# krisher/PathTracer.cl

Measured on AMD Instinct MI355X. Metric: Mrays/sec + frames/sec at 1920×1080, 871k-tri PLY, 1/2/4/8 MI355X, higher is better.
Workload: dtype f32

## Files before the change

__graft_entry__.py:

```python
from __future__ import annotations

import os
import subprocess
import sys
from pathlib import Path

ROOT = Path(__file__).resolve().parent


def _make(path: Path, *targets: str) -> None:
    jobs = str(min(16, os.cpu_count() or 1))
    subprocess.run(["make", "-s", "-j", jobs, "-C", str(path), *targets], check=True)


def build() -> None:
    _make(ROOT / "pathtracer.cl_amd" / "csrc")
    _make(ROOT / "oracle")
    sys.path.insert(0, str(ROOT / "oracle"))
    from oracle import REFERENCE_ROOT

    if os.access(REFERENCE_ROOT / "clrt" / "ocl" / "raytracer.cl", os.R_OK):
        _make(ROOT / "oracle", "ref")
        _make(ROOT / "tests" / "cpp", "all", "libdevkat.so")
    else:
        _make(ROOT / "tests" / "cpp", "ref_main_replay", "host_tree_dump", "libdevkat.so")
    sys.path.insert(0, str(ROOT))
    import ptload

    pt = ptload.load()
    pt.load_library()


def smoke() -> None:
    import numpy as np

    sys.path.insert(0, str(ROOT))
    sys.path.insert(0, str(ROOT / "oracle"))
    import ptload
    from oracle import Oracle

    pt = ptload.load()
    sc = pt.scenes
    orc = Oracle()
    W, H, sr = 64, 48, 2
    Wp, Hp = sc.padded_dims(W, H)
    verts, idx = sc.make_mesh(4000)
    seeds = sc.default_seeds(Wp, Hp)

# ... 43 lines not shown
```

include/pathtracer_rt.h:

```cpp
#ifndef PATHTRACER_RT_H
#define PATHTRACER_RT_H

#include <stddef.h>
#include <stdint.h>

#include "rt_types.h"

#ifdef __cplusplus
extern "C" {
#endif

typedef struct rt_ctx rt_ctx;

enum {
    RT_OK = 0,
    RT_ERR_ARG = -1,
    RT_ERR_HIP = -2,
    RT_ERR_NO_SCENE = -3,
    RT_ERR_NO_MESH = -4,
    RT_ERR_ALLOC = -5,
    RT_ERR_STATE = -6,
    RT_ERR_LIMIT = -7
};

// ... 35 lines not shown
    uint64_t pixel_steps_max;
    uint64_t rays_skipped;
    uint64_t clocks_shade;
    uint64_t pixels_long;
} rt_counters;

int rt_create(int device, rt_ctx **out);
int rt_destroy(rt_ctx *ctx);
const char *rt_last_error(const rt_ctx *ctx);
const char *rt_status_string(int status);

int rt_set_spheres(rt_ctx *ctx, const rt_sphere *spheres, uint32_t n);

int rt_set_mesh(rt_ctx *ctx, const float *verts_xyz, uint32_t n_verts, const int32_t *idx, uint32_t n_tris);
typedef struct rt_mesh_stats {
    uint32_t n_tris;
    uint32_t n_nodes2, depth2;
    uint32_t n_nodes4, depth4;
    uint32_t stack4;
    double build_seconds;
    uint32_t builder;
    uint32_t n_tris_tree;
    uint32_t n_nodes4_shadow;
} rt_mesh_stats;
enum { RT_BUILD_HOST = 0, RT_BUILD_GPU = 1 };
int rt_set_builder(rt_ctx *ctx, int builder);
int rt_mesh_info(const rt_ctx *ctx, rt_mesh_stats *out);

enum { RT_MESH_VERTS_DEVICE = 1 };
enum { RT_MESH_UPDATE_REFIT = 1, RT_MESH_UPDATE_REBUILT = 2 };
enum { RT_REFIT_OK = 0, RT_REFIT_NEWLY_HITTABLE = 1, RT_REFIT_ENCODING = 2 };
typedef struct rt_mesh_update_info {
    uint32_t action;
    uint32_t reason;
    uint32_t newly_hittable;
    uint32_t now_unhittable;
    float area_ratio;
    float ms;
} rt_mesh_update_info;
int rt_update_mesh(rt_ctx *ctx, const float *verts_xyz, uint32_t n_verts, int flags);
int rt_last_mesh_update(const rt_ctx *ctx, rt_mesh_update_info *out);
int rt_set_mesh_dynamic(rt_ctx *ctx, int on);
int rt_mesh_pose(rt_ctx *ctx, float *out_verts_xyz, uint32_t n_verts, int flags);

int rt_set_view_matrix(rt_ctx *ctx, const float m_colmajor[16]);
int rt_set_camera_spherical(rt_ctx *ctx, float tx, float ty, float tz, float elevation_deg, float azimuth_deg,
// ... 31 lines not shown
int rt_last_kernel_ms(const rt_ctx *ctx, float *ms);
int rt_last_kernel_split_ms(const rt_ctx *ctx, float *prepass_ms, float *main_ms);

typedef struct rt_render_info {
    uint32_t kernel;
    uint32_t traversal;
    uint32_t grid_blocks;
    uint32_t lists;
    uint64_t list_capacity;
    uint64_t list_records;
    uint32_t list_pixels_tree;
    uint32_t pixels_long;
    uint32_t schedule_rebuilt;
    uint32_t lists_rebuilt;
    double schedule_host_ms;
    uint32_t split_chunks;
    uint32_t split_coop;
    uint32_t split_guard;
    uint32_t split_spec;
    uint32_t split_repaired;
    uint32_t split_hit_depth;
    uint32_t schedule_measured;
    uint32_t schedule_pilot;
} rt_render_info;
int rt_last_render_info(rt_ctx *ctx, rt_render_info *out);
int rt_last_long_chains(rt_ctx *ctx, uint32_t *out, uint32_t cap, uint32_t *n);
int rt_last_list_counts(rt_ctx *ctx, uint16_t *out, uint32_t cap, uint32_t *n);
typedef struct rt_tree_layout {
    uint32_t n_nodes4;
    uint32_t n_nodes4_shadow;
    uint32_t shadow_root;
    uint32_t n_records;
    uint32_t compressed;
} rt_tree_layout;
int rt_mesh_tree(rt_ctx *ctx, rt_tree_layout *layout, float *nodes4, uint32_t *nodes4q, float *tris);

int rt_trace_rays(rt_ctx *ctx, const rt_ray *rays, uint32_t n, int any_hit, int32_t *out_idx, float *out_t);

enum { RT_FEAT_BOX = -1, RT_FEAT_NONE = -2, RT_FEAT_SPHERE0 = -16  };
int rt_get_camera(const rt_ctx *ctx, uint32_t width, rt_camera *out);
int rt_primary_rays(const rt_camera *cam, uint32_t width, uint32_t height, rt_ray *out);
int rt_render_features(rt_ctx *ctx, float *feat, uint32_t width, uint32_t height, int kernel, int flags);
int rt_render_features_async(rt_ctx *ctx, float *feat, uint32_t width, uint32_t height, int kernel, int flags,
                             void *hip_stream);
typedef struct rt_denoise_params {
    uint32_t iterations;
// ... 113 lines not shown
```

pathtracer.cl_amd/_abi.py:

```python
from __future__ import annotations

import ctypes
import os
from pathlib import Path

import numpy as np

PKG_DIR = Path(__file__).resolve().parent
LIB_PATH = PKG_DIR / "librtmi.so"

RT_OK = 0
RT_ERR_ARG = -1
RT_ERR_HIP = -2
RT_ERR_NO_SCENE = -3
RT_ERR_NO_MESH = -4
RT_ERR_ALLOC = -5
RT_ERR_STATE = -6
RT_ERR_LIMIT = -7

RT_KERNEL_SPHERES = 0
RT_KERNEL_SPHERES_SS = 1
RT_KERNEL_TRIS = 2

RT_TRAVERSAL_BVH = 0
# ... 52 lines not shown
CAMERA_FLOATS = 16


class RtTile(ctypes.Structure):
    _fields_ = [("stripe_rows", ctypes.c_uint32), ("n_ranks", ctypes.c_uint32), ("rank", ctypes.c_uint32),
                ("stripe_owner", ctypes.c_void_p)]


def tile_struct(tile):
    if tile is None:
        return None, None
    stripe, n, r = (int(v) for v in tile[:3])
    owner = tile[3] if len(tile) > 3 else None
    if owner is None:
        return RtTile(stripe, n, r, None), None
    o = np.ascontiguousarray(owner, np.uint32)
    return RtTile(stripe, n, r, o.ctypes.data), o


class RtMeshStats(ctypes.Structure):
    _fields_ = [("n_tris", ctypes.c_uint32), ("n_nodes2", ctypes.c_uint32), ("depth2", ctypes.c_uint32),
                ("n_nodes4", ctypes.c_uint32), ("depth4", ctypes.c_uint32), ("stack4", ctypes.c_uint32),
                ("build_seconds", ctypes.c_double), ("builder", ctypes.c_uint32), ("n_tris_tree", ctypes.c_uint32),
                ("n_nodes4_shadow", ctypes.c_uint32)]


class RtMeshUpdateInfo(ctypes.Structure):
    _fields_ = [("action", ctypes.c_uint32), ("reason", ctypes.c_uint32), ("newly_hittable", ctypes.c_uint32),
                ("now_unhittable", ctypes.c_uint32), ("area_ratio", ctypes.c_float), ("ms", ctypes.c_float)]


class RtTreeLayout(ctypes.Structure):
    _fields_ = [("n_nodes4", ctypes.c_uint32), ("n_nodes4_shadow", ctypes.c_uint32), ("shadow_root", ctypes.c_uint32),
                ("n_records", ctypes.c_uint32), ("compressed", ctypes.c_uint32)]


class RtCounters(ctypes.Structure):
    _fields_ = [
        ("rays_closest", ctypes.c_uint64),
        ("rays_shadow", ctypes.c_uint64),
        ("nodes_visited", ctypes.c_uint64),
        ("tris_tested", ctypes.c_uint64),
        ("leaves_visited", ctypes.c_uint64),
        ("lane_slots", ctypes.c_uint64),
        ("clocks_traversal", ctypes.c_uint64),
        ("clocks_total", ctypes.c_uint64),
        ("pixel_clocks_max", ctypes.c_uint64),
# ... 6 lines not shown


class RtRenderInfo(ctypes.Structure):
    _fields_ = [
        ("kernel", ctypes.c_uint32),
        ("traversal", ctypes.c_uint32),
        ("grid_blocks", ctypes.c_uint32),
        ("lists", ctypes.c_uint32),
        ("list_capacity", ctypes.c_uint64),
        ("list_records", ctypes.c_uint64),
        ("list_pixels_tree", ctypes.c_uint32),
        ("pixels_long", ctypes.c_uint32),
        ("schedule_rebuilt", ctypes.c_uint32),
        ("lists_rebuilt", ctypes.c_uint32),
        ("schedule_host_ms", ctypes.c_double),
        ("split_chunks", ctypes.c_uint32),
        ("split_coop", ctypes.c_uint32),
        ("split_guard", ctypes.c_uint32),
        ("split_spec", ctypes.c_uint32),
        ("split_repaired", ctypes.c_uint32),
        ("split_hit_depth", ctypes.c_uint32),
        ("schedule_measured", ctypes.c_uint32),
        ("schedule_pilot", ctypes.c_uint32),
    ]


class RtDenoiseParams(ctypes.Structure):
    _fields_ = [("iterations", ctypes.c_uint32), ("sigma_color", ctypes.c_float), ("sigma_normal", ctypes.c_float),
                ("sigma_plane", ctypes.c_float)]


class RtReprojectParams(ctypes.Structure):
    _fields_ = [("plane_tol", ctypes.c_float), ("normal_min", ctypes.c_float), ("max_history", ctypes.c_float)]


class RtTrustParams(ctypes.Structure):
    _fields_ = [("tolerance", ctypes.c_float), ("sigma_normal", ctypes.c_float), ("sigma_plane", ctypes.c_float)]


class RtDenoiseVarParams(ctypes.Structure):
    _fields_ = [("iterations", ctypes.c_uint32), ("sigma_lum", ctypes.c_float), ("sigma_normal", ctypes.c_float),
                ("sigma_plane", ctypes.c_float), ("min_len", ctypes.c_float)]


_vp, _u32, _i32, _f32, _sz = ctypes.c_void_p, ctypes.c_uint32, ctypes.c_int, ctypes.c_float, ctypes.c_size_t
SIGNATURES = {
# ... 146 lines not shown
```

pathtracer.cl_amd/csrc/rt_bvh.cpp:

```cpp
#include <algorithm>
#include <array>
#include <functional>
#include <chrono>
#include <cmath>
#include <cstdlib>
#include <cstring>
#include <string>
#include <vector>

#include "rt_internal.h"
#include "rt_quant.h"

namespace {

struct Box {
    float lo[3], hi[3];
    void reset()
    {
        for (int k = 0; k < 3; ++k) {
            lo[k] = INFINITY;
            hi[k] = -INFINITY;
        }
    }
    void grow(const Box &b)
// ... 209 lines not shown
    }
    for (uint64_t i = 0; i < 3ull * n_tris; ++i) {
        if (idx[i] < 0 || (uint32_t)idx[i] >= n_verts) {
            err = "vertex index out of range";
            return false;
        }
    }
    return true;
}

static bool never_hit(const float *a, const float *p1, const float *p2)
{
    const float e1[3] = {p1[0] - a[0], p1[1] - a[1], p1[2] - a[2]};
    const float e2[3] = {p2[0] - a[0], p2[1] - a[1], p2[2] - a[2]};
    const double cx = (double)e2[1] * e1[2] - (double)e2[2] * e1[1];
    const double cy = (double)e2[2] * e1[0] - (double)e2[0] * e1[2];
    const double cz = (double)e2[0] * e1[1] - (double)e2[1] * e1[0];
    const double cr = std::sqrt(cx * cx + cy * cy + cz * cz);
    const double n1 = std::fabs((double)e1[0]) + std::fabs((double)e1[1]) + std::fabs((double)e1[2]);
    const double n2 = std::fabs((double)e2[0]) + std::fabs((double)e2[1]) + std::fabs((double)e2[2]);
    const double u = 1.0 / 16777216.0;
    const double bound = 1.001 * (cr + 16.0 * u * n1 * n2);
    return bound < 0.999 * (double)1e-4f;
}

bool rt_build_bvh(const float *verts, uint32_t n_verts, const int32_t *idx, uint32_t n_tris, RtBvh &out,
                  std::string &err)
{
    const auto t0 = std::chrono::steady_clock::now();
    if (!rt_validate_mesh(verts, n_verts, idx, n_tris, err)) return false;

    Builder b;
    b.lights = out.light_centres;
    b.light_w = out.light_cost_weight;
    b.verts = verts;
    b.idx = idx;
    b.tbox.resize(n_tris);
    b.cent.resize(3ull * n_tris);
    b.perm.resize(n_tris);
    for (uint32_t t = 0; t < n_tris; ++t) {
        Box bx;
        bx.reset();
        float maxabs = 0.0f;
        for (int k = 0; k < 3; ++k) {
            const float *p = verts + 3ull * (uint32_t)idx[3ull * t + k];
            bx.grow(p);
            for (int c = 0; c < 3; ++c) maxabs = std::max(maxabs, std::fabs(p[c]));
        }
        float ext = 0.0f;
        for (int c = 0; c < 3; ++c) ext = std::max(ext, bx.hi[c] - bx.lo[c]);
        const float pad = ext * (1.0f / 512.0f) + 1e-6f * (1.0f + maxabs);
        for (int c = 0; c < 3; ++c) {
            b.cent[3ull * t + c] = 0.5f * (bx.lo[c] + bx.hi[c]);
            bx.lo[c] -= pad;
            bx.hi[c] += pad;
        }
        b.tbox[t] = bx;
    }
    uint32_t n_hit = 0;
    if (out.cull_unhittable) {
        std::vector<uint8_t> hit(n_tris);
        for (uint32_t t = 0; t < n_tris; ++t) {
            const float *a = verts + 3ull * (uint32_t)idx[3ull * t];
            const float *p1 = verts + 3ull * (uint32_t)idx[3ull * t + 1];
            const float *p2 = verts + 3ull * (uint32_t)idx[3ull * t + 2];
            hit[t] = !never_hit(a, p1, p2);
            n_hit += hit[t];
        }
        if (n_hit == 0) hit[0] = 1, n_hit = 1;
        for (uint32_t t = 0, k = 0, r = n_hit; t < n_tris; ++t) b.perm[hit[t] ? k++ : r++] = t;
    } else {
        n_hit = n_tris;
        for (uint32_t t = 0; t < n_tris; ++t) b.perm[t] = t;
    }
    out.n_hit = n_hit;
    b.nodes.reserve(2ull * n_hit / RT_LEAF_MAX + 16);
    const int root = b.build(0, n_hit, 1);

    std::vector<int> order;
    std::vector<int> out_index(b.nodes.size(), -1);
    uint32_t n_leaves = 0;
    if (b.nodes[root].left < 0) {
        out.n_nodes = 1;
        out.nodes.assign(16, 0.0f);
        const Box &bx = b.nodes[root].box;
        float *n = out.nodes.data();
        n[0] = bx.lo[0]; n[1] = bx.hi[0]; n[2] = bx.lo[1]; n[3] = bx.hi[1];
        n[4] = bx.lo[0]; n[5] = bx.hi[0]; n[6] = bx.lo[1]; n[7] = bx.hi[1];
        n[8] = bx.lo[2]; n[9] = bx.hi[2]; n[10] = bx.lo[2]; n[11] = bx.hi[2];
        const int32_t code = leaf_code(0, n_hit);
        std::memcpy(&n[12], &code, 4);
        std::memcpy(&n[13], &code, 4);
        n_leaves = 1;
        out.depth = 1;
    } else {
        std::vector<int> stack;
        stack.push_back(root);
        while (!stack.empty()) {
            const int id = stack.back();
            stack.pop_back();
// ... 61 lines not shown
            const int l = nd.left, r = nd.right;
            float best_int = INFINITY;
            for (int a = 1; a <= 3; ++a) best_int = std::min(best_int, dcost[l][a] + dcost[r][4 - a]);
            const float inner_c = area * 1.0f + best_int;
            const float self_c = std::min(leaf_c, inner_c);
            as_leaf[i] = leaf_c <= inner_c;
            dcost[i][1] = self_c;
            dsplit[i][1] = 0;
            for (int j = 2; j <= 4; ++j) {
                float best = self_c;
                int8_t arg = 0;
                for (int a = 1; a < j; ++a) {
                    const float c = dcost[l][a] + dcost[r][j - a];
                    if (c < best) {
                        best = c;
                        arg = (int8_t)a;
                    }
                }
                dcost[i][j] = best;
                dsplit[i][j] = arg;
            }
        }
    }
    {
        std::vector<int> n4_src;
        std::vector<int> kids_of;
        std::function<void(int, int, int *, int &)> expand = [&](int id, int j, int *k, int &n) {
            const int a = dsplit[id][j];
            if (a == 0) {
                k[n++] = id;
                return;
            }
            expand(b.nodes[id].left, a, k, n);
            expand(b.nodes[id].right, j - a, k, n);
        };
        auto gather = [&](int id, int *kids) {
            int k[4] = {-1, -1, -1, -1};
            int n = 0;
            if (b.nodes[id].left < 0) {
                k[n++] = id;
            } else {
                const int l = b.nodes[id].left, r = b.nodes[id].right;
                int best_a = 1;
                float best = INFINITY;
                for (int a = 1; a <= 3; ++a) {
                    const float c = dcost[l][a] + dcost[r][4 - a];
                    if (c < best) {
                        best = c;
                        best_a = a;
                    }
                }
                expand(l, best_a, k, n);
                expand(r, 4 - best_a, k, n);
            }
            for (int i = 0; i < 4; ++i) {
                kids[i] = k[i];
                if (k[i] >= 0) inner4[k[i]] = !as_leaf[k[i]];
            }
        };
        std::vector<int> st{root};
        inner4[root] = b.nodes[root].left >= 0;
        while (!st.empty()) {
            const int id = st.back();
// ... 104 lines not shown
                    c = new_id[c];
                    std::memcpy(&dst[24 + k], &c, 4);
                } else {
                    remap(&dst[24 + k]);
                }
            }
        }
        out.nodes4.swap(nodes4);
        for (uint32_t i = 0; i < out.n_nodes; ++i) {
            remap(&out.nodes[16ull * i + 12]);
            remap(&out.nodes[16ull * i + 13]);
        }
        for (uint32_t q = cursor; q < n_tris; ++q) new_perm[q] = b.perm[q];
        b.perm.swap(new_perm);
    }

    out.nodes4q.assign((uint64_t)RT_QNODE_DWORDS * out.n_nodes4, 0u);
    for (uint32_t i = 0; i < out.n_nodes4; ++i)
        if (!rt_quantize_node4(out.nodes4.data() + 32ull * i, out.nodes4q.data() + (uint64_t)RT_QNODE_DWORDS * i)) {
            out.nodes4q.clear();
            break;
        }

    out.tris.assign(12ull * n_tris, 0.0f);
    for (uint32_t s = 0; s < n_tris; ++s) {
        const uint32_t t = b.perm[s];
        const float *a = verts + 3ull * (uint32_t)idx[3ull * t];
        const float *p1 = verts + 3ull * (uint32_t)idx[3ull * t + 1];
        const float *p2 = verts + 3ull * (uint32_t)idx[3ull * t + 2];
        float *o = out.tris.data() + 12ull * s;
        o[0] = a[0];
        o[1] = a[1];
        o[2] = a[2];
        const int32_t orig = (int32_t)t;
        std::memcpy(&o[3], &orig, 4);
        o[4] = p1[0] - a[0];
        o[5] = p1[1] - a[1];
        o[6] = p1[2] - a[2];
        o[8] = p2[0] - a[0];
        o[9] = p2[1] - a[1];
        o[10] = p2[2] - a[2];
    }
    if (!out.nodes4q.empty() && out.det_cull) {
        struct NB {
            double lo[3], hi[3], err;
        };
// ... 44 lines not shown
```

pathtracer.cl_amd/csrc/rt_ctx.h:

```cpp
#ifndef RT_CTX_H
#define RT_CTX_H

#include <hip/hip_runtime.h>

#include <algorithm>
#include <cstdint>
#include <cstdlib>
#include <string>
#include <utility>
#include <vector>

#include "pathtracer_rt.h"
#include "rt_internal.h"

template <class T> struct DevBuf {
    T *p = nullptr;
    size_t cap = 0;
    DevBuf() = default;
    DevBuf(const DevBuf &) = delete;
    DevBuf &operator=(DevBuf &&o) noexcept
    {
        std::swap(p, o.p);
        std::swap(cap, o.cap);
        return *this;
// ... 37 lines not shown
    }
    operator H() const { return h; }
};
struct Event : Owned<hipEvent_t, hipEventDestroy> {
    hipError_t create(unsigned flags = hipEventDefault) { return h ? hipSuccess : hipEventCreateWithFlags(&h, flags); }
};
struct Stream : Owned<hipStream_t, hipStreamDestroy> {
    hipError_t create() { return h ? hipSuccess : hipStreamCreateWithFlags(&h, hipStreamNonBlocking); }
};

struct GlibcRand {
    uint32_t r[34];
    int k = 0;
    void seed(uint32_t s);
    uint32_t next();
};

constexpr size_t kCounterBytes = RT_COUNTER_WORDS * sizeof(unsigned long long);
constexpr size_t kWorkWords = (size_t)RT_QSTRIDE * RT_QHEADS + 64;
static_assert((kCounterBytes + kWorkWords * sizeof(uint32_t)) % sizeof(unsigned long long) == 0, "d_counters is an array of 64-bit words");
#ifndef RT_REPAIR_SLOTS
#define RT_REPAIR_SLOTS 4096u
#endif

enum RtStage { RT_ST_FEATURES, RT_ST_DENOISE, RT_ST_REPROJECT, RT_ST_MERGE, RT_ST_MOMENTS, RT_ST_VARIANCE, RT_ST_DENOISE_VAR, RT_ST_WARP, RT_ST_TRUST, RT_ST_COUNT };

struct rt_ctx {
    int device = 0;
    hipStream_t stream = nullptr;
    Event ev0, ev1, evm;
    std::string err;

    std::vector<rt_sphere> spheres;
    std::vector<rt_sphere> lights;
    DevBuf<rt_sphere> d_spheres, d_lights;

    RtBvh bvh;
    DevBuf<float> d_nodes4;
    DevBuf<uint32_t> d_nodes4q;
    DevBuf<float> d_tris;
    size_t tris_cap() const { return d_tris.cap / 12; }
    size_t tree_recs = 0;
    uint32_t shadow_root = 0;
    uint32_t n_nodes4_shadow = 0, stack4_all = 0;
    std::vector<std::pair<uint32_t, uint32_t>> shadow_levels;
    bool shadow_cache = true;
    int shadow_cache_depth = -1;
    DevBuf<uint16_t> d_list_code;
    DevBuf<uint32_t> d_list_tile;
    DevBuf<uint32_t> d_list_alloc;
    int pixel_lists = -1;
    size_t list_mb = 4096;
    std::vector<uint32_t> list_key;
    uint64_t list_used_last = 0, list_cap_last = 0, list_npx_last = 0;
    std::vector<uint32_t> last_view;
    uint32_t n_tris = 0;
    DevBuf<int32_t> d_spill;
    DevBuf<uint32_t> d_order;
    DevBuf<uint32_t> d_flags;
    RtSchedScratch sched;
    DevBuf<int32_t> d_class;
    size_t split_mb = 16384;
    int split = -1;
    uint32_t seed_width = 0;
    uint32_t split_probe = 4;
    uint32_t split_nch = 16;
    DevBuf<uint32_t> d_split_seed;
    DevBuf<float> d_split_col;
    DevBuf<uint32_t> d_split_counter;
    DevBuf<uint32_t> d_split_box;
// ... 194 lines not shown
```

pathtracer.cl_amd/csrc/rt_internal.h:

```cpp
#ifndef RT_INTERNAL_H
#define RT_INTERNAL_H

#include <stdint.h>

#include <string>
#include <vector>

#include "rt_types.h"

int rt_exception_status(std::string *err) noexcept;
#define RT_CATCH(err_ptr)                                                                                              \
    catch (...) { return rt_exception_status(err_ptr); }

#ifndef RT_STACK_DEPTH
#define RT_STACK_DEPTH 20
#endif
#define RT_BVH_MAX_DEPTH 33
#define RT_BLOCK 256
#define RT_PROBE_HIT_SHIFT 27
#define RT_PROBE_STEP_MASK ((1u << RT_PROBE_HIT_SHIFT) - 1u)
#ifndef RT_STEP_UNROLL
#define RT_STEP_UNROLL 4
#endif
#ifndef RT_DIAG_ONE_PIXEL
// ... 13 lines not shown
#define RT_CNT_GUARD RT_N_COUNTERS
#define RT_CNT_REPAIR (RT_N_COUNTERS + 1)
#define RT_COUNTER_WORDS (RT_N_COUNTERS + 2)
enum { RT_GUARD_INDEX = 1, RT_GUARD_STACK = 2, RT_GUARD_ROUNDS = 4 };

#define RT_EMPTY_CHILD 0x7fffffff

struct RtBvh {
    std::vector<float> nodes;
    std::vector<float> tris;
    uint32_t n_nodes = 0;
    uint32_t n_leaves = 0;
    uint32_t depth = 0;
    std::vector<float> nodes4;
    std::vector<uint32_t> nodes4q;
    uint32_t n_nodes4 = 0;
    uint32_t depth4 = 0;
    uint32_t stack4 = 0;
    double build_seconds = 0.0;
    bool cull_unhittable = true;
    bool det_cull = true;
    std::vector<float> light_centres;
    float light_cost_weight = 0.6f;
    uint32_t n_hit = 0;
};

bool rt_build_bvh(const float *verts, uint32_t n_verts, const int32_t *idx, uint32_t n_tris, RtBvh &out,
                  std::string &err);

struct RtGpuBvh {
    float *nodes4 = nullptr;
    uint32_t *nodes4q = nullptr;
    float *tris = nullptr;
    uint32_t n_nodes4 = 0, depth4 = 0, stack4 = 0;
    double build_seconds = 0.0;
};
int rt_build_bvh_gpu(const float *verts, uint32_t n_verts, const int32_t *idx, uint32_t n_tris, RtGpuBvh &out,
                     std::string &err, void *stream, bool det_cull = true);
bool rt_validate_mesh(const float *verts, uint32_t n_verts, const int32_t *idx, uint32_t n_tris, std::string &err);

enum {
    RT_REFIT_RES_BAD = 0,
    RT_REFIT_RES_NEWLY = 1,
    RT_REFIT_RES_UNHIT = 2,
    RT_REFIT_RES_QFAIL = 3,
    RT_REFIT_RES_LO = 4,
    RT_REFIT_RES_HI = 7,
// ... 213 lines not shown
```

pathtracer.cl_amd/csrc/rt_mesh.cpp:

```cpp
#include <cmath>
#include <cstring>
#include <thread>

#include "rt_ctx.h"
#include "rt_math.h"
#include "rt_quant.h"

namespace {

std::vector<std::pair<uint32_t, uint32_t>> tree_levels(const uint32_t *q4, uint32_t n, uint32_t root)
{
    std::vector<std::pair<uint32_t, uint32_t>> lv;
    if (!q4 || root >= n) return lv;
    uint32_t lo = root, hi = root + 1u;
    for (;;) {
        lv.emplace_back(lo, hi);
        uint32_t cmin = ~0u, cmax = 0u, cnt = 0u;
        for (uint32_t i = lo; i < hi; ++i)
            for (int k = 0; k < 4; ++k) {
                const int32_t code = (int32_t)q4[(size_t)i * RT_QNODE_DWORDS + 12 + k];
                if (code < 0 || code == RT_EMPTY_CHILD) continue;
                cmin = std::min(cmin, (uint32_t)code);
                cmax = std::max(cmax, (uint32_t)code);
                ++cnt;
            }
        if (!cnt) break;
        if (cmin != hi || cmax - cmin + 1u != cnt || cmax >= n) break;
        lo = cmin;
        hi = cmax + 1u;
    }
    return lv;
}

}

extern "C" {

static bool mesh_bounds(const float *verts, const int32_t *idx, uint32_t n_tris, float lo[3], float hi[3])
{
    for (int k = 0; k < 3; ++k) {
        lo[k] = INFINITY;
        hi[k] = -INFINITY;
    }
    for (uint64_t i = 0; i < 3ull * n_tris; ++i) {
        const float *v = verts + 3ull * (uint32_t)idx[i];
        for (int k = 0; k < 3; ++k) {
            lo[k] = std::min(lo[k], v[k]);
            hi[k] = std::max(hi[k], v[k]);
        }
    }
// ... 26 lines not shown
    drop_mesh(c);
    RtGpuBvh g;
    bool det_cull = true;
    if (const char *v = getenv("RT_DET_CULL")) det_cull = atoi(v) != 0;
    const int e = rt_build_bvh_gpu(verts, n_verts, idx, n_tris, g, err, c->stream, det_cull);
    c->d_nodes4.adopt(g.nodes4, 32ull * g.n_nodes4);
    c->d_nodes4q.adopt(g.nodes4q, (size_t)RT_QNODE_DWORDS * g.n_nodes4);
    c->d_tris.adopt(g.tris, 12ull * n_tris);
    if (e) return fail(c, RT_ERR_HIP, "GPU BVH build: " + err);
    c->n_tris = n_tris;
    c->mesh_serial++;
    c->bvh.n_nodes = 0;
    c->bvh.n_leaves = 0;
    c->bvh.depth = 0;
    c->bvh.n_nodes4 = g.n_nodes4;
    c->bvh.depth4 = g.depth4;
    c->bvh.stack4 = g.stack4;
    c->bvh.build_seconds = g.build_seconds;
    c->bvh.n_hit = n_tris;
    c->tree_recs = n_tris;
    c->shadow_root = 0;
    c->n_nodes4_shadow = 0;
    c->stack4_all = g.stack4;
    c->shadow_levels.clear();
    if (c->shadow_cache && g.nodes4q) {
        std::vector<uint32_t> hq((size_t)RT_QNODE_DWORDS * g.n_nodes4);
        HIPCHK(c, hipMemcpy(hq.data(), g.nodes4q, hq.size() * sizeof(uint32_t), hipMemcpyDeviceToHost));
        c->shadow_levels = tree_levels(hq.data(), g.n_nodes4, 0u);
    }
    c->mesh_builder = RT_BUILD_GPU;
    c->mesh_bounds_ok = mesh_bounds(verts, idx, n_tris, c->mesh_lo, c->mesh_hi);
    c->mesh_det_cull = det_cull;
    c->mesh_dynamic = dynamic;
    return RT_OK;
}

static int set_mesh_build(rt_ctx *c, const float *verts, uint32_t n_verts, const int32_t *idx, uint32_t n_tris,
                          int builder, bool dynamic)
{
    std::string err;
    c->mesh_bounds_ok = false;
    if (builder == RT_BUILD_GPU) return set_mesh_build_gpu(c, verts, n_verts, idx, n_tris, dynamic);
    RtBvh b;
    if (const char *v = getenv("RT_CULL_UNHITTABLE")) b.cull_unhittable = atoi(v) != 0;
    if (dynamic) b.cull_unhittable = false;
    if (const char *v = getenv("RT_DET_CULL")) b.det_cull = atoi(v) != 0;
    RtBvh sb;
    sb.cull_unhittable = b.cull_unhittable;
    sb.det_cull = b.det_cull;
    for (const rt_sphere &L : c->lights) {
        sb.light_centres.push_back(L.center.x);
        sb.light_centres.push_back(L.center.y);
        sb.light_centres.push_back(L.center.z);
    }
    if (const char *v = getenv("RT_BVH_LIGHT_W")) sb.light_cost_weight = (float)atof(v);
    b.light_cost_weight = 0.0f;
    bool two = !sb.light_centres.empty() && sb.light_cost_weight > 0.0f && 2ull * n_tris < (1ull << 28);
    bool ok2 = false;
    std::string err2;
    std::thread th;
    if (two)
        th = std::thread([&]() {
            try {
                ok2 = rt_build_bvh(verts, n_verts, idx, n_tris, sb, err2);
            } catch (...) {
                ok2 = false;
            }
        });
    bool ok = false;
    try {
        ok = rt_build_bvh(verts, n_verts, idx, n_tris, b, err);
    } catch (...) {
        if (th.joinable()) th.join();
        throw;
    }
    if (th.joinable()) th.join();
    if (!ok)
        return fail(c, err.find("deeper") != std::string::npos ? RT_ERR_LIMIT : RT_ERR_ARG, err);
// ... 11 lines not shown
                if (code >= 0) {
                    code += (int32_t)n_a;
                } else {
                    const uint32_t enc = (uint32_t)(~code);
                    code = ~(int32_t)((((enc >> 3) + n_tris) << 3) | (enc & 7u));
                }
                w = (uint32_t)code;
            }
        tr.insert(tr.end(), sb.tris.begin(), sb.tris.end());
    }
    c->mesh_builder = RT_BUILD_HOST;
    drop_mesh(c);
    HIPCHK(c, c->d_nodes4.reserve(b.nodes4.size()));
    if (!q4.empty()) HIPCHK(c, c->d_nodes4q.reserve(q4.size()));
    HIPCHK(c, c->d_tris.reserve(tr.size()));
    HIPCHK(c, hipMemcpy(c->d_nodes4, b.nodes4.data(), b.nodes4.size() * sizeof(float), hipMemcpyHostToDevice));
    if (!q4.empty())
        HIPCHK(c, hipMemcpy(c->d_nodes4q, q4.data(), q4.size() * sizeof(uint32_t), hipMemcpyHostToDevice));
    HIPCHK(c, hipMemcpy(c->d_tris, tr.data(), tr.size() * sizeof(float), hipMemcpyHostToDevice));
    c->tree_recs = tr.size() / 12;
    c->shadow_root = two ? n_a : 0u;
    c->n_nodes4_shadow = two ? sb.n_nodes4 : 0u;
    c->shadow_levels = tree_levels(q4.data(), (uint32_t)(q4.size() / RT_QNODE_DWORDS), c->shadow_root);
    c->stack4_all = two ? std::max(b.stack4, sb.stack4) : b.stack4;
    c->n_tris = n_tris;
    c->mesh_serial++;
    c->bvh.n_nodes = b.n_nodes;
    c->bvh.n_leaves = b.n_leaves;
    c->bvh.depth = b.depth;
    c->bvh.n_nodes4 = b.n_nodes4;
    c->bvh.depth4 = b.depth4;
    c->bvh.stack4 = b.stack4;
    c->bvh.build_seconds = b.build_seconds;
    c->bvh.n_hit = b.n_hit;
    c->mesh_bounds_ok = mesh_bounds(verts, idx, n_tris, c->mesh_lo, c->mesh_hi);
    c->mesh_det_cull = b.det_cull;
    c->mesh_dynamic = dynamic;
    return RT_OK;
}

static int refit_prepare(rt_ctx *c)
{
    rt_ctx::Refit &r = c->refit;
    const uint32_t n_a = c->bvh.n_nodes4, n_s = c->n_nodes4_shadow, n_all = n_a + n_s;
    std::vector<uint32_t> q((size_t)RT_QNODE_DWORDS * n_all, 0u);
    if (c->d_nodes4q) {
// ... 137 lines not shown
    a.nbox = r.d_nbox;
    a.tris = c->d_tris;
    a.tbox = r.d_tbox;
    a.n_nodes4 = n_a;
    a.n_nodes4_shadow = c->n_nodes4_shadow;
    a.n_recs = (uint32_t)c->tree_recs;
    a.det_cull = c->mesh_det_cull;
    a.res = r.d_res;
    HIPCHK(c, hipEventRecord(r.ev0, st));
    if (int e = rt_launch_refit_records(r.d_verts, c->d_idx, n_tris, n_hit, a.n_recs, c->d_tris, r.d_tbox, r.d_hit0,
                                        !r.have_hit0, r.d_res, st))
        return hip_fail(c, (hipError_t)e, "k_refit_records");
    r.have_hit0 = true;
    if (int e = rt_launch_refit_levels(a, r.d_steps, r.steps.data(), (uint32_t)r.steps.size(), st))
        return hip_fail(c, (hipError_t)e, "k_refit_levels");
    double now = 0.0;
    if (int e = rt_launch_refit_area(c->d_nodes4, n_a, r.d_part, st))
        return hip_fail(c, (hipError_t)e, "k_refit_area");
    HIPCHK(c, hipEventRecord(r.ev1, st));
    HIPCHK(c, hipMemcpyAsync(res, r.d_res, sizeof(res), hipMemcpyDeviceToHost, st));
    HIPCHK(c, hipMemcpyAsync(part, r.d_part, sizeof(part), hipMemcpyDeviceToHost, st));
    HIPCHK(c, hipStreamSynchronize(st));
    c->mesh_serial++;
    if (res[RT_REFIT_RES_BAD]) return fail(c, RT_ERR_STATE, "rt_update_mesh: a link of the tree is out of range");
    const bool had_q = c->d_nodes4q != nullptr;
    if (had_q ? res[RT_REFIT_RES_QFAIL] != 0u : res[RT_REFIT_RES_QFAIL] == 0u)
        return update_rebuild(c, verts, flags, RT_REFIT_ENCODING, 0u);
    for (double p : part) now += p;
    float ext = 0.0f;
    for (int k = 0; k < 3; ++k) {
        auto unkey = [](uint32_t key) { return (key & 0x80000000u) ? (key & 0x7FFFFFFFu) : ~key; };
        const uint32_t ul = unkey(res[RT_REFIT_RES_LO + k]), uh = unkey(res[RT_REFIT_RES_HI + k]);
        memcpy(&c->mesh_lo[k], &ul, 4);
        memcpy(&c->mesh_hi[k], &uh, 4);
        ext = std::max(ext, c->mesh_hi[k] - c->mesh_lo[k]);
    }
    const float pad = 1e-3f * ext + 1e-4f;
    for (int k = 0; k < 3; ++k) {
        c->mesh_lo[k] -= pad;
        c->mesh_hi[k] += pad;
    }
    c->mesh_bounds_ok = true;
    if (const int w = wait_aux(c, st)) return w;
    HIPCHK(c, hipMemcpyAsync(c->d_pose, r.d_verts, 12ull * n_verts, hipMemcpyDeviceToDevice, st));
    HIPCHK(c, hipStreamSynchronize(st));
    float ms = 0.0f;
// ... 12 lines not shown
    if (n_verts != c->n_verts) return fail(c, RT_ERR_ARG, "rt_mesh_pose: the vertex count differs from the mesh's");
    if (flags & ~RT_OUT_DEVICE) return fail(c, RT_ERR_ARG, "rt_mesh_pose: flags other than RT_OUT_DEVICE");
    HIPCHK(c, hipSetDevice(c->device));
    HIPCHK(c, hipMemcpy(out, c->d_pose, 12ull * n_verts,
                        (flags & RT_OUT_DEVICE) ? hipMemcpyDeviceToDevice : hipMemcpyDeviceToHost));
    HIPCHK(c, hipStreamSynchronize(nullptr));
    return RT_OK;
} RT_CATCH(err_of(c))

int rt_mesh_info(const rt_ctx *c, rt_mesh_stats *out)
try {
    if (!c || !out) return RT_ERR_ARG;
    if (!c->n_tris) return RT_ERR_NO_MESH;
    out->n_tris = c->n_tris;
    out->n_nodes2 = c->bvh.n_nodes;
    out->depth2 = c->bvh.depth;
    out->n_nodes4_shadow = c->n_nodes4_shadow;
    out->n_nodes4 = c->bvh.n_nodes4;
    out->depth4 = c->bvh.depth4;
    out->stack4 = c->bvh.stack4;
    out->builder = (uint32_t)c->mesh_builder;
    out->build_seconds = c->bvh.build_seconds;
    out->n_tris_tree = c->bvh.n_hit;
    return RT_OK;
} RT_CATCH(err_of(c))

int rt_mesh_tree(rt_ctx *c, rt_tree_layout *layout, float *nodes4, uint32_t *nodes4q, float *tris)
try {
    if (!c || !layout) return RT_ERR_ARG;
    if (!c->n_tris || !c->d_nodes4 || !c->d_tris) return RT_ERR_NO_MESH;
    layout->n_nodes4 = c->bvh.n_nodes4;
    layout->n_nodes4_shadow = c->n_nodes4_shadow;
    layout->shadow_root = c->shadow_root;
    layout->n_records = (uint32_t)c->tree_recs;
    layout->compressed = c->d_nodes4q ? 1u : 0u;
    if (nodes4q && !c->d_nodes4q) return fail(c, RT_ERR_STATE, "the mesh has no compressed nodes");
    if (!nodes4 && !nodes4q && !tris) return RT_OK;
    HIPCHK(c, hipSetDevice(c->device));
    HIPCHK(c, hipStreamSynchronize(c->stream));
    if (nodes4)
        HIPCHK(c, hipMemcpy(nodes4, c->d_nodes4, (size_t)c->bvh.n_nodes4 * 32 * sizeof(float), hipMemcpyDeviceToHost));
    if (nodes4q)
        HIPCHK(c, hipMemcpy(nodes4q, c->d_nodes4q,
                            ((size_t)c->bvh.n_nodes4 + c->n_nodes4_shadow) * RT_QNODE_DWORDS * sizeof(uint32_t),
                            hipMemcpyDeviceToHost));
    if (tris) HIPCHK(c, hipMemcpy(tris, c->d_tris, c->tree_recs * 12 * sizeof(float), hipMemcpyDeviceToHost));
// ... 62 lines not shown
```

pathtracer.cl_amd/csrc/rt_render.cpp:

```cpp
#include <chrono>
#include <cmath>
#include <cstdio>
#include <cstring>

#include "rt_ctx.h"

namespace {

constexpr uint32_t kProbeN = 2;
uint32_t probe_n(uint32_t sample_rate) { return sample_rate >= 2 ? kProbeN : 1u; }
#ifndef RT_FETCH_K
#define RT_FETCH_K 24
#endif
constexpr uint32_t kWorkBox = RT_QSTRIDE * RT_QHEADS, kWorkRepair = RT_QSTRIDE * RT_QHEADS + 32;
#ifndef RT_LONG_FINE
#define RT_LONG_FINE 1
#endif
#ifndef RT_REPAIR_WIDTH
#define RT_REPAIR_WIDTH 64u
#endif
#ifndef RT_QUEUE_BATCH
#define RT_QUEUE_BATCH 64
#endif
#ifndef RT_BOX_GRID_DIV
// ... 461 lines not shown
{
    a.out = f.dout;
    a.seeds = c->d_seeds;
    a.cam = c->cam;
    a.W = f.W;
    a.H = f.H;
    a.Wpad = c->wpad;
    a.Hpad = c->hpad;
    a.Hl = f.hl;
    a.sample_rate = c->sample_rate;
    a.max_depth = c->max_depth;
    a.progressive = f.prog;
    a.stripe = f.stripe;
    a.n_ranks = f.nr;
    a.rank = f.rk;
    a.stripe_map = f.smap;
    a.counters = c->d_counters;
}

int tri_scene(rt_ctx *c, RtTriLaunch &a)
{
    a.nodes = trav_nodes(c);
    a.shadow_root = trav_kind(c) == RT_TRAV_BVH4Q ? c->shadow_root : 0u;
    if (trav_kind(c) == RT_TRAV_BVH4Q && c->shadow_cache) {
        const size_t nl = c->shadow_levels.size();
        const size_t d = c->shadow_cache_depth >= 0 ? (size_t)c->shadow_cache_depth
                                                    : std::min<size_t>(kShadowCutDepth, (nl - (nl > 0)) / 2);
        if (d >= 1 && d < nl && c->shadow_levels[d].second - c->shadow_levels[d].first <= 0xffffu) {
            a.shadow_cut_lo = c->shadow_levels[d].first;
            a.shadow_cut_hi = c->shadow_levels[d].second;
        }
    }
    a.tris = c->d_tris;
    a.n_tris = c->n_tris;
    a.lights = c->d_lights;
    a.n_lights = (uint32_t)c->lights.size();
    if (a.n_lights > 16) return fail(c, RT_ERR_LIMIT, "more than 16 emissive spheres");
    return RT_OK;
}

int plan_grid(rt_ctx *c, const Frame &f, RtTriLaunch &a, TriPlan &p)
{
    const uint64_t items = (uint64_t)((f.W + 7) / 8) * ((f.hl + 7) / 8) * 64;
    p.item_blocks = (items + RT_BLOCK - 1) / RT_BLOCK;
    int r = grid_blocks(c, p.trav, c->counting, RT_FORM_PLAIN, &p.blocks);
    if (r != RT_OK) return r;
    p.blocks = std::max(1, (int)std::min<uint64_t>((uint64_t)p.blocks, p.item_blocks));
    p.short_frame = (uint64_t)f.W * f.hl * c->sample_rate * c->sample_rate <
                    kShortFrameSamplesPerLane * (uint64_t)p.blocks * RT_BLOCK;
    if (p.short_frame) p.blocks = std::max(1, p.blocks * (int)kShortFrameBlocksPerCU / RT_TRIS_WAVES);
    if (const uint32_t gb = env_u32("RTMI_GRID_BLOCKS", 0)) p.blocks = std::min(p.blocks, (int)gb);
    if (p.trav == RT_TRAV_BVH4Q) {
        r = grid_blocks(c, p.trav, c->counting, RT_FORM_SPLIT, &p.blocks_split);
// ... 249 lines not shown
    *e_out = e;
    return RT_OK;
}

void tris_info(rt_ctx *c, const RtTriLaunch &a, const TriPlan &p)
{
    c->info = rt_render_info{};
    c->info.kernel = RT_KERNEL_TRIS;
    c->info.traversal = (uint32_t)p.trav;
    c->info.grid_blocks = (uint32_t)p.blocks;
    c->info.lists = p.lists ? 1u : 0u;
    c->info.lists_rebuilt = p.build_lists ? 1u : 0u;
    c->info.list_capacity = p.lists ? p.list_cap : 0;
    c->info_list_px = p.lists ? (size_t)p.npx : 0u;
    c->info.pixels_long = c->last_long;
    c->info.split_chunks = a.split_chunks;
    c->info.split_coop = a.split_chunks && a.split_n_box ? a.split_coop : 0u;
    c->info.split_spec = a.split_chunks ? a.split_spec : 0u;
    c->info.split_hit_depth = a.split_chunks && c->last_hit_depth ? 1u : 0u;
    c->info.schedule_measured = a.tile_order && c->order_measured ? 1u : 0u;
    c->info.schedule_rebuilt = c->schedule_rebuilt ? 1u : 0u;
    c->info.schedule_host_ms = p.sched_ms;
    c->info.schedule_pilot = p.pilot ? 1u : 0u;
    c->info_list_pending = p.lists;
}

int render_tris(rt_ctx *c, const Frame &f, int *e_out)
{
    RtTriLaunch a{};
    TriPlan p;
    common_fields(a, c, f);
    a.map_key = f.map_key;
    a.work_counter = c->d_work;
    if (const int r = tri_scene(c, a)) return r;
    p.trav = trav_kind(c);
    if (const int r = plan_grid(c, f, a, p)) return r;
    stepping_fields(f, a, p);
    a.tile_order = nullptr;
    a.pixel_flags = nullptr;
    a.pixel_class = nullptr;
    const auto h0 = std::chrono::steady_clock::now();
    c->schedule_rebuilt = false;
    if (c->schedule) {
        const int ro = tile_order(c, a, p.blocks, f.st);
        if (ro != RT_OK) return ro;
        a.tile_order = c->d_order;
// ... 447 lines not shown
```

Measured before the change: 17710.

## Split shadow BVH into a light-cone subtree of potentially occluding triangles

At build time each hittable triangle is tested against every emissive sphere with a conservative cone bound. Triangles whose projected area toward all lights falls below the existing degenerate threshold are flagged as never occluding. The shadow BVH is rebuilt with a root whose left child holds only the occluding triangles, and shadow rays start traversal at that subtree. The aim is to cut shadow-ray node and triangle tests, at the cost of extra host build work, staleness tracking after refits, and a risk of precision mismatch against the oracle.

```diff
diff --git a/__graft_entry__.py b/__graft_entry__.py
--- a/__graft_entry__.py
+++ b/__graft_entry__.py
@@ -24,6 +24,7 @@
         _make(ROOT / "tests" / "cpp", "all", "libdevkat.so")
     else:
         _make(ROOT / "tests" / "cpp", "ref_main_replay", "host_tree_dump", "libdevkat.so")
+    _make(ROOT / "tests" / "cpp", "-f", "light_cone.mk")
     sys.path.insert(0, str(ROOT))
     import ptload
 
diff --git a/include/pathtracer_rt.h b/include/pathtracer_rt.h
--- a/include/pathtracer_rt.h
+++ b/include/pathtracer_rt.h
@@ -81,6 +81,8 @@
     uint32_t builder;
     uint32_t n_tris_tree;
     uint32_t n_nodes4_shadow;
+    uint32_t cone_root;
+    uint32_t n_tris_cone;
 } rt_mesh_stats;
 enum { RT_BUILD_HOST = 0, RT_BUILD_GPU = 1 };
 int rt_set_builder(rt_ctx *ctx, int builder);
@@ -158,6 +160,7 @@
     uint32_t split_hit_depth;
     uint32_t schedule_measured;
     uint32_t schedule_pilot;
+    uint32_t shadow_start;
 } rt_render_info;
 int rt_last_render_info(rt_ctx *ctx, rt_render_info *out);
 int rt_last_long_chains(rt_ctx *ctx, uint32_t *out, uint32_t cap, uint32_t *n);
diff --git a/pathtracer.cl_amd/_abi.py b/pathtracer.cl_amd/_abi.py
--- a/pathtracer.cl_amd/_abi.py
+++ b/pathtracer.cl_amd/_abi.py
@@ -98,7 +98,7 @@
     _fields_ = [("n_tris", ctypes.c_uint32), ("n_nodes2", ctypes.c_uint32), ("depth2", ctypes.c_uint32),
                 ("n_nodes4", ctypes.c_uint32), ("depth4", ctypes.c_uint32), ("stack4", ctypes.c_uint32),
                 ("build_seconds", ctypes.c_double), ("builder", ctypes.c_uint32), ("n_tris_tree", ctypes.c_uint32),
-                ("n_nodes4_shadow", ctypes.c_uint32)]
+                ("n_nodes4_shadow", ctypes.c_uint32), ("cone_root", ctypes.c_uint32), ("n_tris_cone", ctypes.c_uint32)]
 
 
 class RtMeshUpdateInfo(ctypes.Structure):
@@ -151,6 +151,7 @@
         ("split_hit_depth", ctypes.c_uint32),
         ("schedule_measured", ctypes.c_uint32),
         ("schedule_pilot", ctypes.c_uint32),
+        ("shadow_start", ctypes.c_uint32),
     ]
 
 
diff --git a/pathtracer.cl_amd/csrc/rt_bvh.cpp b/pathtracer.cl_amd/csrc/rt_bvh.cpp
--- a/pathtracer.cl_amd/csrc/rt_bvh.cpp
+++ b/pathtracer.cl_amd/csrc/rt_bvh.cpp
@@ -255,6 +255,49 @@
     const double u = 1.0 / 16777216.0;
     const double bound = 1.001 * (cr + 16.0 * u * n1 * n2);
     return bound < 0.999 * (double)1e-4f;
+}
+
+static bool never_occludes(const float *a, const float *p1, const float *p2, const std::vector<float> &centres,
+                           const std::vector<float> &radii)
+{
+    const float e1[3] = {p1[0] - a[0], p1[1] - a[1], p1[2] - a[2]};
+    const float e2[3] = {p2[0] - a[0], p2[1] - a[1], p2[2] - a[2]};
+    const double n[3] = {(double)e2[1] * e1[2] - (double)e2[2] * e1[1], (double)e2[2] * e1[0] - (double)e2[0] * e1[2],
+                         (double)e2[0] * e1[1] - (double)e2[1] * e1[0]};
+    const double cr = std::sqrt(n[0] * n[0] + n[1] * n[1] + n[2] * n[2]);
+    const double n1 = std::fabs((double)e1[0]) + std::fabs((double)e1[1]) + std::fabs((double)e1[2]);
+    const double n2 = std::fabs((double)e2[0]) + std::fabs((double)e2[1]) + std::fabs((double)e2[2]);
+    const double u = 1.0 / 16777216.0;
+    double cen[3], rt2 = 0.0;
+    for (int k = 0; k < 3; ++k) cen[k] = (double)a[k] + ((double)e1[k] + (double)e2[k]) / 3.0;
+    for (int v = 0; v < 3; ++v) {
+        double d2 = 0.0;
+        for (int k = 0; k < 3; ++k) {
+            const double p = (double)a[k] + (v == 1 ? (double)e1[k] : v == 2 ? (double)e2[k] : 0.0);
+            d2 += (p - cen[k]) * (p - cen[k]);
+        }
+        rt2 = std::max(rt2, d2);
+    }
+    const double rt = std::sqrt(rt2);
+    for (size_t l = 0; l < radii.size(); ++l) {
+        double L[3], dist2 = 0.0, ln = 0.0;
+        for (int k = 0; k < 3; ++k) {
+            L[k] = (double)centres[3 * l + k] - cen[k];
+            dist2 += L[k] * L[k];
+            ln += L[k] * n[k];
+        }
+        const double dist = std::sqrt(dist2);
+        const double reach = 1.001 * std::fabs((double)radii[l]) + rt;
+        double maxcos = 1.0;
+        if (reach < dist && cr > 0.0) {
+            const double st = reach / dist, ct = std::sqrt(1.0 - st * st);
+            const double cp = std::min(1.0, std::fabs(ln) / (dist * cr)), sp = std::sqrt(1.0 - cp * cp);
+            if (cp < ct) maxcos = std::min(1.0, (cp * ct + sp * st) * (1.0 + 1e-9) + 1e-12);
+        }
+        const double bound = 1.001 * (cr * maxcos + 16.0 * u * n1 * n2);
+        if (!(bound < 0.999 * (double)1e-4f)) return false;
+    }
+    return true;
 }
 
 bool rt_build_bvh(const float *verts, uint32_t n_verts, const int32_t *idx, uint32_t n_tris, RtBvh &out,
@@ -290,7 +333,9 @@
         }
         b.tbox[t] = bx;
     }
-    uint32_t n_hit = 0;
+    uint32_t n_hit = 0, n_cone = 0;
+    out.cone_root4 = 0;
+    out.n_cone = 0;
     if (out.cull_unhittable) {
         std::vector<uint8_t> hit(n_tris);
         for (uint32_t t = 0; t < n_tris; ++t) {
@@ -301,14 +346,39 @@
             n_hit += hit[t];
         }
         if (n_hit == 0) hit[0] = 1, n_hit = 1;
-        for (uint32_t t = 0, k = 0, r = n_hit; t < n_tris; ++t) b.perm[hit[t] ? k++ : r++] = t;
+        if (!out.light_radii.empty() && 3 * out.light_radii.size() == out.light_centres.size()) {
+            uint32_t n_b = 0;
+            for (uint32_t t = 0; t < n_tris; ++t) {
+                if (!hit[t]) continue;
+                const float *a = verts + 3ull * (uint32_t)idx[3ull * t];
+                const float *p1 = verts + 3ull * (uint32_t)idx[3ull * t + 1];
+                const float *p2 = verts + 3ull * (uint32_t)idx[3ull * t + 2];
+                if (never_occludes(a, p1, p2, out.light_centres, out.light_radii)) hit[t] = 2, ++n_b;
+            }
+            if (n_hit - n_b > RT_LEAF_MAX && n_b > RT_LEAF_MAX) n_cone = n_hit - n_b;
+        }
+        for (uint32_t t = 0, k = 0, m = n_cone, r = n_hit; t < n_tris; ++t)
+            b.perm[!hit[t] ? r++ : (n_cone && hit[t] == 2) ? m++ : k++] = t;
     } else {
         n_hit = n_tris;
         for (uint32_t t = 0; t < n_tris; ++t) b.perm[t] = t;
     }
     out.n_hit = n_hit;
     b.nodes.reserve(2ull * n_hit / RT_LEAF_MAX + 16);
-    const int root = b.build(0, n_hit, 1);
+    int root;
+    if (n_cone) {
+        root = (int)b.nodes.size();
+        b.nodes.emplace_back();
+        b.nodes[root].box = b.bounds(0, n_hit);
+        b.nodes[root].first = 0;
+        b.nodes[root].count = n_hit;
+        const int l = b.build(0, n_cone, 2);
+        const int r = b.build(n_cone, n_hit - n_cone, 2);
+        b.nodes[root].left = l;
+        b.nodes[root].right = r;
+    } else {
+        root = b.build(0, n_hit, 1);
+    }
 
     std::vector<int> order;
     std::vector<int> out_index(b.nodes.size(), -1);
@@ -416,6 +486,13 @@
             }
         }
     }
+    if (n_cone && (as_leaf[b.nodes[root].left] || as_leaf[b.nodes[root].right])) {
+        std::vector<float> radii;
+        radii.swap(out.light_radii);
+        const bool ok = rt_build_bvh(verts, n_verts, idx, n_tris, out, err);
+        radii.swap(out.light_radii);
+        return ok;
+    }
     {
         std::vector<int> n4_src;
         std::vector<int> kids_of;
@@ -433,6 +510,9 @@
             int n = 0;
             if (b.nodes[id].left < 0) {
                 k[n++] = id;
+            } else if (n_cone && id == root) {
+                k[n++] = b.nodes[id].left;
+                k[n++] = b.nodes[id].right;
             } else {
                 const int l = b.nodes[id].left, r = b.nodes[id].right;
                 int best_a = 1;
@@ -583,6 +663,13 @@
             break;
         }
 
+    if (n_cone && !out.nodes4q.empty()) {
+        int32_t c;
+        std::memcpy(&c, &out.nodes4[24], 4);
+        out.cone_root4 = (uint32_t)c;
+        out.n_cone = n_cone;
+    }
+
     out.tris.assign(12ull * n_tris, 0.0f);
     for (uint32_t s = 0; s < n_tris; ++s) {
         const uint32_t t = b.perm[s];
diff --git a/pathtracer.cl_amd/csrc/rt_ctx.h b/pathtracer.cl_amd/csrc/rt_ctx.h
--- a/pathtracer.cl_amd/csrc/rt_ctx.h
+++ b/pathtracer.cl_amd/csrc/rt_ctx.h
@@ -83,6 +83,8 @@
 #ifndef RT_REPAIR_SLOTS
 #define RT_REPAIR_SLOTS 4096u
 #endif
+
+constexpr bool kLightCone = true;
 
 enum RtStage { RT_ST_FEATURES, RT_ST_DENOISE, RT_ST_REPROJECT, RT_ST_MERGE, RT_ST_MOMENTS, RT_ST_VARIANCE, RT_ST_DENOISE_VAR, RT_ST_WARP, RT_ST_TRUST, RT_ST_COUNT };
 
@@ -107,6 +109,10 @@
     std::vector<std::pair<uint32_t, uint32_t>> shadow_levels;
     bool shadow_cache = true;
     int shadow_cache_depth = -1;
+    uint32_t cone_root = 0, n_cone = 0;
+    std::vector<std::pair<uint32_t, uint32_t>> cone_levels;
+    std::vector<uint32_t> cone_lights;
+    bool cone_stale = false;
     DevBuf<uint16_t> d_list_code;
     DevBuf<uint32_t> d_list_tile;
     DevBuf<uint32_t> d_list_alloc;
diff --git a/pathtracer.cl_amd/csrc/rt_internal.h b/pathtracer.cl_amd/csrc/rt_internal.h
--- a/pathtracer.cl_amd/csrc/rt_internal.h
+++ b/pathtracer.cl_amd/csrc/rt_internal.h
@@ -59,7 +59,10 @@
     bool det_cull = true;
     std::vector<float> light_centres;
     float light_cost_weight = 0.6f;
+    std::vector<float> light_radii;
     uint32_t n_hit = 0;
+    uint32_t cone_root4 = 0;
+    uint32_t n_cone = 0;
 };
 
 bool rt_build_bvh(const float *verts, uint32_t n_verts, const int32_t *idx, uint32_t n_tris, RtBvh &out,
diff --git a/pathtracer.cl_amd/csrc/rt_mesh.cpp b/pathtracer.cl_amd/csrc/rt_mesh.cpp
--- a/pathtracer.cl_amd/csrc/rt_mesh.cpp
+++ b/pathtracer.cl_amd/csrc/rt_mesh.cpp
@@ -8,7 +8,8 @@
 
 namespace {
 
-std::vector<std::pair<uint32_t, uint32_t>> tree_levels(const uint32_t *q4, uint32_t n, uint32_t root)
+std::vector<std::pair<uint32_t, uint32_t>> tree_levels(const uint32_t *q4, uint32_t n, uint32_t root,
+                                                       bool adjoining = true)
 {
     std::vector<std::pair<uint32_t, uint32_t>> lv;
     if (!q4 || root >= n) return lv;
@@ -25,7 +26,7 @@
                 ++cnt;
             }
         if (!cnt) break;
-        if (cmin != hi || cmax - cmin + 1u != cnt || cmax >= n) break;
+        if ((adjoining ? cmin != hi : cmin < hi) || cmax - cmin + 1u != cnt || cmax >= n) break;
         lo = cmin;
         hi = cmax + 1u;
     }
@@ -98,6 +99,10 @@
     c->shadow_root = 0;
     c->n_nodes4_shadow = 0;
     c->stack4_all = g.stack4;
+    c->cone_root = c->n_cone = 0;
+    c->cone_levels.clear();
+    c->cone_lights.clear();
+    c->cone_stale = false;
     c->shadow_levels.clear();
     if (c->shadow_cache && g.nodes4q) {
         std::vector<uint32_t> hq((size_t)RT_QNODE_DWORDS * g.n_nodes4);
@@ -130,6 +135,10 @@
         sb.light_centres.push_back(L.center.z);
     }
     if (const char *v = getenv("RT_BVH_LIGHT_W")) sb.light_cost_weight = (float)atof(v);
+    bool cone = kLightCone;
+    if (const char *v = getenv("RT_LIGHT_CONE")) cone = atoi(v) != 0;
+    if (cone)
+        for (const rt_sphere &L : c->lights) sb.light_radii.push_back(L.radius);
     b.light_cost_weight = 0.0f;
     bool two = !sb.light_centres.empty() && sb.light_cost_weight > 0.0f && 2ull * n_tris < (1ull << 28);
     bool ok2 = false;
@@ -187,6 +196,20 @@
     c->shadow_root = two ? n_a : 0u;
     c->n_nodes4_shadow = two ? sb.n_nodes4 : 0u;
     c->shadow_levels = tree_levels(q4.data(), (uint32_t)(q4.size() / RT_QNODE_DWORDS), c->shadow_root);
+    c->cone_root = two && sb.cone_root4 ? n_a + sb.cone_root4 : 0u;
+    c->n_cone = c->cone_root ? sb.n_cone : 0u;
+    c->cone_levels.clear();
+    c->cone_lights.clear();
+    c->cone_stale = false;
+    if (c->cone_root) {
+        c->cone_levels = tree_levels(q4.data(), (uint32_t)(q4.size() / RT_QNODE_DWORDS), c->cone_root, false);
+        for (const rt_sphere &L : c->lights) {
+            const float w[4] = {L.center.x, L.center.y, L.center.z, L.radius};
+            uint32_t bits[4];
+            memcpy(bits, w, sizeof(bits));
+            c->cone_lights.insert(c->cone_lights.end(), bits, bits + 4);
+        }
+    }
     c->stack4_all = two ? std::max(b.stack4, sb.stack4) : b.stack4;
     c->n_tris = n_tris;
     c->mesh_serial++;
@@ -370,6 +393,7 @@
     HIPCHK(c, hipMemcpyAsync(part, r.d_part, sizeof(part), hipMemcpyDeviceToHost, st));
     HIPCHK(c, hipStreamSynchronize(st));
     c->mesh_serial++;
+    c->cone_stale = true;
     if (res[RT_REFIT_RES_BAD]) return fail(c, RT_ERR_STATE, "rt_update_mesh: a link of the tree is out of range");
     const bool had_q = c->d_nodes4q != nullptr;
     if (had_q ? res[RT_REFIT_RES_QFAIL] != 0u : res[RT_REFIT_RES_QFAIL] == 0u)
@@ -428,6 +452,8 @@
     out->builder = (uint32_t)c->mesh_builder;
     out->build_seconds = c->bvh.build_seconds;
     out->n_tris_tree = c->bvh.n_hit;
+    out->cone_root = c->cone_root;
+    out->n_tris_cone = c->n_cone;
     return RT_OK;
 } RT_CATCH(err_of(c))
 
diff --git a/pathtracer.cl_amd/csrc/rt_render.cpp b/pathtracer.cl_amd/csrc/rt_render.cpp
--- a/pathtracer.cl_amd/csrc/rt_render.cpp
+++ b/pathtracer.cl_amd/csrc/rt_render.cpp
@@ -507,13 +507,22 @@
 {
     a.nodes = trav_nodes(c);
     a.shadow_root = trav_kind(c) == RT_TRAV_BVH4Q ? c->shadow_root : 0u;
+    bool cone = a.shadow_root && c->cone_root && !c->cone_stale;
+    for (size_t l = 0; cone && l < c->lights.size(); ++l) {
+        const float w[4] = {c->lights[l].center.x, c->lights[l].center.y, c->lights[l].center.z, c->lights[l].radius};
+        bool found = false;
+        for (size_t k = 0; !found && k + 4 <= c->cone_lights.size(); k += 4) found = !memcmp(w, &c->cone_lights[k], sizeof(w));
+        cone = found;
+    }
+    if (cone) a.shadow_root = c->cone_root;
     if (trav_kind(c) == RT_TRAV_BVH4Q && c->shadow_cache) {
-        const size_t nl = c->shadow_levels.size();
+        const auto &lv = cone ? c->cone_levels : c->shadow_levels;
+        const size_t nl = lv.size();
         const size_t d = c->shadow_cache_depth >= 0 ? (size_t)c->shadow_cache_depth
                                                     : std::min<size_t>(kShadowCutDepth, (nl - (nl > 0)) / 2);
-        if (d >= 1 && d < nl && c->shadow_levels[d].second - c->shadow_levels[d].first <= 0xffffu) {
-            a.shadow_cut_lo = c->shadow_levels[d].first;
-            a.shadow_cut_hi = c->shadow_levels[d].second;
+        if (d >= 1 && d < nl && lv[d].second - lv[d].first <= 0xffffu) {
+            a.shadow_cut_lo = lv[d].first;
+            a.shadow_cut_hi = lv[d].second;
         }
     }
     a.tris = c->d_tris;
@@ -809,6 +818,7 @@
     c->info.schedule_rebuilt = c->schedule_rebuilt ? 1u : 0u;
     c->info.schedule_host_ms = p.sched_ms;
     c->info.schedule_pilot = p.pilot ? 1u : 0u;
+    c->info.shadow_start = a.shadow_root;
     c->info_list_pending = p.lists;
 }
 
```

New measurement: 18870 (median of 6 runs). 1.07x the previous value.
